# ash-shar/Long-Tail-GAN

Measured on AMD Instinct MI355X. Metric: train users/sec at BATCH_SIZE=100, higher is better.
Workload: dtype bf16

## Files before the change

long-tail-gan_amd/csrc/ltg_fast_small.h:

```cpp
#pragma once


template <bool BF>
__global__ __launch_bounds__(NT) void fk_dec1(int B, int I, int H, const float* __restrict__ h2, const float* __restrict__ Wp1t,
                                              const float* __restrict__ bp1, float* __restrict__ logits) {
    __shared__ __attribute__((aligned(16))) float lds[Rg16::LDS_FLOATS];
    const LtgTile2 tl = xcd_tile2();
    const int m0 = tl.y * 16, n0 = tl.x * 16;
    auto a_ld = [=] __device__(int, int m, int k) { return ltg_ld4(h2 + (size_t)m * H + k); };
    auto b_ld = [=] __device__(int, int k, int n) { return ltg_ld4(Wp1t + (size_t)n * H + k); };
    auto xf = [=] __device__(ltg_f32x4 v, int, int, int) { return BF ? ltg_bf16r4(v) : v; };
    const float biasv = bp1[min(n0 + (int)(threadIdx.x & 15), I - 1)];
    auto epi = [=] __device__(int, int m, int n, float v, bool ok) {
        if (ok) logits[(size_t)m * I + n] = v + biasv;
    };
    if constexpr (BF) ltg_rgemm<1, 1, 1, 1, 4, 5, true>(B, I, H, m0, n0, a_ld, xf, b_ld, xf, epi, lds);
    else ltg_rgemm<1, 1, 1, 1, 4, 10>(B, I, H, m0, n0, a_ld, xf, b_ld, xf, epi, lds);
}

__device__ __forceinline__ void block_red4(float& a, float& b, float& c, float& mx, float (*red)[NT / 64]) {
#pragma unroll
    for (int o = 32; o > 0; o >>= 1) {
        a += __shfl_xor(a, o);
        b += __shfl_xor(b, o);
        c += __shfl_xor(c, o);
        mx = fmaxf(mx, __shfl_xor(mx, o));
    }
    const int w = threadIdx.x >> 6;
    if ((threadIdx.x & 63) == 0) {
        red[0][w] = a;
        red[1][w] = b;
        red[2][w] = c;
        red[3][w] = mx;
    }
    __syncthreads();
    a = red[0][0] + red[0][1] + red[0][2] + red[0][3];
    b = red[1][0] + red[1][1] + red[1][2] + red[1][3];
    c = red[2][0] + red[2][1] + red[2][2] + red[2][3];
    mx = fmaxf(fmaxf(red[3][0], red[3][1]), fmaxf(red[3][2], red[3][3]));
    __syncthreads();
}

__global__ __launch_bounds__(NT) void fk_row_dlogits(int B, int I, const int32_t* __restrict__ indptr, const int32_t* __restrict__ indices,
                                                     const float* __restrict__ values, const float* __restrict__ logits,
                                                     const float* __restrict__ kl_rows, const float* __restrict__ y, int nf,
                                                     const int32_t* __restrict__ cnt, float lam, const int32_t* __restrict__ f_row,
                                                     const int32_t* __restrict__ f_gen, const int32_t* __restrict__ f_pop,
                                                     float* __restrict__ dlog, float* __restrict__ lse, float* __restrict__ rowout) {
    __shared__ float s_l[RD_MAXI];
    __shared__ float s_x[RD_MAXI];
    __shared__ uint8_t s_s[RD_MAXI];
    __shared__ float red[4][NT / 64];
    static_assert(NT / 64 == 4, "block_red4 adds four wave partials");
    const int b = blockIdx.x, tid = threadIdx.x;
    const float* row = logits + (size_t)b * I;
    constexpr int PER = RD_MAXI / NT;
    const int e0 = indptr[b], e1 = indptr[b + 1];
    float v[PER];
#pragma unroll
    for (int j = 0; j < PER; ++j) {
        const int i = tid + NT * j;
        v[j] = row[min(i, I - 1)];
    }
    constexpr int RD_U = 4;
    int tg0[RD_U], tr0[RD_U], tp0[RD_U];
#pragma unroll
    for (int u = 0; u < RD_U; ++u) tg0[u] = tr0[u] = tp0[u] = -1;
    if (nf > 0) {
#pragma unroll
        for (int u = 0; u < RD_U; ++u) {
            const int q = min(tid + u * NT, nf - 1);
            tg0[u] = f_gen[q];
            tr0[u] = f_row[q];
            tp0[u] = f_pop[q];
        }
    }
    const int cntv = cnt[0];
    const float klb = kl_rows[b];
    int it0 = -1;
    float x0 = 1.f;
    if (e0 + tid < e1) {
        it0 = indices[e0 + tid];
        if (values) x0 = values[e0 + tid];
    }
    float sy = 0.f;
    for (int q0 = tid; q0 < nf; q0 += RD_U * NT) {
        float ty[RD_U];
#pragma unroll
        for (int u = 0; u < RD_U; ++u) ty[u] = y[min(q0 + u * NT, nf - 1)];
#pragma unroll
        for (int u = 0; u < RD_U; ++u)
            if (q0 + u * NT < nf) sy += ty[u];
    }
    float mx = -INFINITY;
#pragma unroll
    for (int j = 0; j < PER; ++j) {
        const int i = tid + NT * j;
        if (i < I) {
            s_l[i] = v[j];
            s_x[i] = 0.f;
            s_s[i] = 0;
            mx = fmaxf(mx, v[j]);
        } else v[j] = -INFINITY;
    }
    __syncthreads();
    float xl = 0.f, nx = 0.f;
    if (it0 >= 0) {
        s_x[it0] = x0;
        xl += x0 * s_l[it0];
        nx += x0;
    }
    for (int e = e0 + tid + NT; e < e1; e += NT) {
        const int it = indices[e];
        const float x = values ? values[e] : 1.f;
        s_x[it] = x;
        xl += x * s_l[it];
        nx += x;
    }
#pragma unroll
    for (int u = 0; u < RD_U; ++u)
        if (tid + u * NT < nf && tr0[u] == b && tg0[u] >= 0 && tg0[u] < I && tp0[u] >= 0) s_s[tg0[u]] = 1;
    for (int q0 = tid + RD_U * NT; q0 < nf; q0 += RD_U * NT) {
        int tg[RD_U], tr[RD_U], tp[RD_U];
#pragma unroll
        for (int u = 0; u < RD_U; ++u) {
            const int q = min(q0 + u * NT, nf - 1);
            tg[u] = f_gen[q];
            tr[u] = f_row[q];
            tp[u] = f_pop[q];
        }
#pragma unroll
        for (int u = 0; u < RD_U; ++u)
            if (q0 + u * NT < nf && tr[u] == b && tg[u] >= 0 && tg[u] < I && tp[u] >= 0) s_s[tg[u]] = 1;
    }
    block_red4(xl, nx, sy, mx, red);
    float s = 0.f, psu = 0.f, zero = 0.f, m2 = 0.f;
#pragma unroll
    for (int j = 0; j < PER; ++j) {
        const int i = tid + NT * j;
        const float ex = expf(v[j] - mx);
        s += ex;
        psu += (i < I && s_s[i]) ? ex : 0.f;
    }
    block_red4(s, psu, zero, m2, red);
    const float l = mx + logf(s);
    const float ps = psu / s;
    const float invB = 1.f / (float)B, invs = 1.f / s;
    const float c = cntv > 0 ? lam / (float)cntv * sy : 0.f;
    const float alpha = nx * invB + c * ps;
#pragma unroll
    for (int j = 0; j < PER; ++j) {
        const int i = tid + NT * j;
        if (i < I) {
            const float p = expf(v[j] - mx) * invs;
            dlog[(size_t)b * I + i] = p * alpha - s_x[i] * invB - (s_s[i] ? c * p : 0.f);
        }
    }
    if (tid == 0) {
        lse[b] = l;
        float* o = rowout + (size_t)b * 4;
        o[0] = -xl + nx * l;
        o[1] = ps;
        o[2] = klb;
        o[3] = sy;
    }
}

constexpr int DH2_NT = 512;
template <bool BF>
__global__ __launch_bounds__(DH2_NT) void fk_dh2(int B, int I, int H, const float* __restrict__ dlog, const float* __restrict__ Wp1t,
                                             const float* __restrict__ h2, float* __restrict__ da2) {
    __shared__ __attribute__((aligned(16))) float lds[LtgRg<1, 1, 1, 1, 8>::LDS_FLOATS];
    const LtgTile2 tl = xcd_tile2();
    const int m0 = tl.y * 16, n0 = tl.x * 16;
    auto a_ld = [=] __device__(int, int m, int k) { return ltg_ld4(dlog + (size_t)m * I + k); };
    auto b_ld = [=] __device__(int, int k, int n) { return ltg_ld4s(Wp1t + (size_t)k * H + n, H); };
    auto xf = [=] __device__(ltg_f32x4 v, int, int, int) { return BF ? ltg_bf16r4(v) : v; };
    const float t = h2[(size_t)min(m0 + (int)(threadIdx.x >> 4), B - 1) * H + min(n0 + (int)(threadIdx.x & 15), H - 1)];
    auto epi = [=] __device__(int, int m, int n, float v, bool ok) {
        if (ok) da2[(size_t)m * H + n] = v * (1.f - t * t);
    };
    if constexpr (BF) ltg_rgemm<1, 1, 1, 1, 8, 4, true>(B, H, I, m0, n0, a_ld, xf, b_ld, xf, epi, lds);
    else ltg_rgemm<1, 1, 1, 1, 8, 8>(B, H, I, m0, n0, a_ld, xf, b_ld, xf, epi, lds);
}

struct WgTensors {
    float *W, *mW, *vW, *b, *mb, *vb;
};
struct WgWhere {
    float *p, *m, *v;
    bool vec;
};
struct WgRegs {
    ltg_f32x4 p, m, v;
};
#ifndef LTG_TAIL_BN
#define LTG_TAIL_BN 32
#endif
template <bool RND, bool ONES_L>
__device__ __forceinline__ void wgrad_adam_tile(int K, int Min, int Nin, const float* __restrict__ Lm, int ldl, const float* __restrict__ Rm,
                                                int ldr, WgTensors T, int ldw, AdamC ad, int m0, int n0, float* __restrict__ lds, unsigned dead = 0u) {
    const int M = ONES_L ? Min + 1 : Min, N = ONES_L ? Nin : Nin + 1;
    auto a_ld = [=] __device__(int, int m, int k) {
        ltg_f32x4 v;
#pragma unroll
        for (int j = 0; j < 4; ++j) v[j] = Lm[(size_t)min(k + j, K - 1) * ldl + min(m, Min - 1)];
        return v;
    };
    auto a_xf = [=] __device__(ltg_f32x4 x, int, int m, int k) {
        ltg_f32x4 v;
#pragma unroll
        for (int j = 0; j < 4; ++j) v[j] = k + j < K ? ((ONES_L && m == Min) ? 1.f : (RND ? ltg_bf16r(x[j]) : x[j])) : 0.f;
        return v;
    };
    auto b_ld = [=] __device__(int, int k, int n) {
        ltg_f32x4 v;
// ... 214 lines not shown
```

long-tail-gan_amd/csrc/ltg_kernels.hip:

```cpp
#include <hip/hip_runtime.h>
#include <math.h>
#include <stdint.h>

#include "../../include/ltg.h"
#include "ltg_gemm.h"
#include "ltg_rng.h"

namespace {

constexpr int NT = 256;

struct AdamC {
    float lr_t, b1, b2, eps;
};

__device__ __forceinline__ float adam_move(const float p, const float lm, const float v, const float eps) {
#ifdef LTG_ADAM_IEEE
    return p - lm / (sqrtf(v) + eps);
#else
    return __builtin_fmaf(-lm, __builtin_amdgcn_rcpf(__builtin_amdgcn_sqrtf(v) + eps), p);
#endif
}
__device__ __forceinline__ void adam1(float& p, float& m, float& v, const float g, const float lr_t, const AdamC& c) {
    m = __builtin_fmaf(c.b1, m, (1.f - c.b1) * g);
// ... 105 lines not shown
#include "ltg_diversify.h"

inline size_t align_up(size_t x, size_t a = 256) { return (x + a - 1) / a * a; }

inline bool stream_ok(const ltg_config* cfg, const ltg_gen_state* gen, int rows) {
    return gen->wp1t_bf16 && cfg->precision == LTG_PREC_BF16 && cfg->n_items >= 8192 && (cfg->n_items % 8) == 0 && rows <= 128 && cfg->h_enc <= ST_KP &&
           (cfg->h_enc % 4) == 0;
}
inline bool dw_stream_ok(int H) { return (H % 4) == 0 && H > 576 && H <= 640; }
constexpr int DH2_NH = 2;
inline int dh2_stream_chunk1(int I);
inline int dh2_stream_chunk(int I) { return DH2_NH * dh2_stream_chunk1(I); }
inline int dh2_stream_chunk1(int I) {
    int c = (I + 255) / 256;
    c = (c + ST_BN - 1) / ST_BN * ST_BN;
    return c < 4 * ST_BN ? 4 * ST_BN : c;
}

inline int dh2_kchunk(int I) {
    int chunk = (I + 63) / 64;
    chunk = (chunk + 31) / 32 * 32;
    if (chunk < 256) chunk = 256;
    return chunk;
}

inline size_t gq0_rows(const ltg_config* cfg, int ) { return (size_t)cfg->n_items; }

constexpr int RD_MAXI = 4096;
struct Workspace {
    float *rowpart, *segpart, *nb, *Pb, *scal, *dlog, *part, *dh2, *da2, *dmlv, *da1, *gq0;
    int32_t* slotmap;
    float *A1, *A3, *y, *ds, *lrow, *dpre1, *dpre3, *slab;
    float *spart, *G3, *rowout, *xd;
    uint8_t* A1_8;
    uint8_t *A1T_8, *dpre3_8, *dpre3T_8, *dpre1T_8, *ET_8;
    unsigned short* dA1T_16;
    int np8;
    float* wsp;
    size_t bytes;
};
inline int d_slab_stride(int P) { return (P + 1 + 3) & ~3; }

constexpr int FT_BM = 64, FT_NT = 512;
constexpr int FT_KP1_MAX = 4;
inline int ft_lda(int h12) { return ((h12 + 31) & ~31) + 4; }
inline size_t ft_lds_bytes(int h12) { return ((size_t)FT_BM * ft_lda(h12) + 4 * FT_BM) * sizeof(float); }
inline size_t ft_wsp_triples(int h0, int h1, int h2, int h3) {
    const size_t kp1 = (h0 + 31) / 32, kp3 = (h1 + h2 + 31) / 32;
    return (size_t)((h1 + 15) / 16) * kp1 + (size_t)((h2 + 15) / 16) * kp1 + (size_t)((h3 + 15) / 16) * kp3;
}
inline size_t ft_wsp_bytes(int h0, int h1, int h2, int h3) { return ft_wsp_triples(h0, h1, h2, h3) * 3 * 1024; }
inline bool ft_wsp_capable(const ltg_config* c) {
    return (c->tuning & 262144) == 0 && c->d_precision == LTG_PREC_FP32 && !(c->d_h0 >= 512 && c->d_h1 + c->d_h2 >= 512 && c->d_h3 >= 128) && c->d_h0 >= 4 &&
           c->d_h0 <= 32 * FT_KP1_MAX && (c->d_h0 % 4) == 0 && c->d_h1 >= 1 && c->d_h2 >= 1 && c->d_h3 >= 1 && c->d_h3 <= 320 &&
           ft_lds_bytes(c->d_h1 + c->d_h2) <= (size_t)160 * 1024;
}
Workspace carve(const ltg_config* cfg, int max_rows, int max_pairs, char* base) {
    Workspace w;
    size_t off = 0;
    auto take = [&](size_t nfloat) {
        float* p = reinterpret_cast<float*>(base + off);
        off += align_up(nfloat * sizeof(float));
        return p;
    };
    const size_t R = (size_t)max_rows, I = (size_t)cfg->n_items, H = (size_t)cfg->h_enc, Z = (size_t)cfg->z_dim;
    const size_t P = (size_t)max_pairs, h12 = (size_t)cfg->d_h1 + cfg->d_h2, h3 = (size_t)cfg->d_h3;
// ... 16 lines not shown
    w.da1 = take(R * H);
    w.gq0 = take((size_t)(gq0_rows(cfg, max_rows) + ENC0_BIAS_PARTS) * H);
    w.slotmap = reinterpret_cast<int32_t*>(take(I));
    w.A1 = take(P * h12);
    w.A3 = take(P * h3);
    w.y = take(P);
    w.ds = take(P);
    w.lrow = take(P);
    w.dpre1 = take(P * h12);
    w.dpre3 = take(P * h3);
    {
        const DLayout L = d_layout(cfg->d_h0, cfg->d_h1, cfg->d_h2, cfg->d_h3);
        const size_t ks = (P + D_KCHUNK - 1) / D_KCHUNK;
        w.slab = take(ks * (size_t)d_slab_stride(L.off[8]));
    }
    w.spart = take((((h3 + 31) / 32) + 1) * P);
    w.G3 = take(P * h3);
    w.rowout = take(R * 4);
    w.xd = take(I <= (size_t)RD_MAXI ? R * I : 1);
    w.A1_8 = reinterpret_cast<uint8_t*>(take((P * h12 + 3) / 4));
    {
        const bool f8 = cfg->d_precision == LTG_PREC_FP8;
        const size_t np = ((P + 127) / 128 * 128), h0 = (size_t)cfg->d_h0;
        auto take8 = [&](size_t nbytes) { return reinterpret_cast<uint8_t*>(take(f8 ? (nbytes + 3) / 4 : 1)); };
        w.np8 = (int)np;
        w.A1T_8 = take8((h12 + 1) * np);
        w.dA1T_16 = reinterpret_cast<unsigned short*>(take8(2 * h12 * np));
        w.dpre3_8 = take8(P * h3);
        w.dpre3T_8 = take8(h3 * np);
        w.dpre1T_8 = take8(h12 * np);
        w.ET_8 = take8(2 * (h0 + 1) * np);
    }
    w.wsp = take(ft_wsp_capable(cfg) ? ft_wsp_bytes(cfg->d_h0, cfg->d_h1, cfg->d_h2, cfg->d_h3) / sizeof(float) : 1);
    w.bytes = off;
    return w;
}

inline AdamC make_adam(const ltg_config* cfg, int t) {
    AdamC a;
    const double b1 = cfg->beta1, b2 = cfg->beta2;
    a.lr_t = (float)((double)cfg->lr * sqrt(1.0 - pow(b2, (double)t)) / (1.0 - pow(b1, (double)t)));
    a.b1 = cfg->beta1;
    a.b2 = cfg->beta2;
    a.eps = cfg->adam_eps;
    return a;
}

struct Probe {
    const ltg_probe* p;
    hipStream_t st;
    inline void before(int id) const {
        if (p && p->kernel_id == id && p->ev_start) (void)hipEventRecord((hipEvent_t)p->ev_start, st);
    }
    inline void after(int id) const {
        if (p && p->kernel_id == id && p->ev_stop) (void)hipEventRecord((hipEvent_t)p->ev_stop, st);
    }
};
#define LTG_PROBED(pr, id, stmt) \
    do {                         \
        (pr).before(id);         \
        stmt;                    \
        (pr).after(id);          \
    } while (0)

inline int check_launch() { return hipGetLastError() == hipSuccess ? LTG_OK : LTG_ELAUNCH; }
inline void clear_errors() { (void)hipGetLastError(); }
// ... 75 lines not shown
    if (fast_on(cfg)) {
        LTG_PROBED(pr, LTG_K_ENC0_FWD,
                   hipLaunchKernelGGL(fk_enc0_fwd, dim3((H / 4 + 63) / 64, R + (end_wait.word ? 1 : 0)), dim3(ENC_NT), xd ? (size_t)I * sizeof(float) : 0, st, H, I, bt->indptr,
                                      bt->indices, bt->values, o->drop_keep, o->keep_prob, cfg->seed, o->rng_step, gen->p[0], gen->p[4], acts->h1,
                                      acts->row_scale, bt->row_norm2, cfg->item_lo, Ig_of(cfg), pre_only, xd, o->rows_per_step, started, end_wait));
        return;
    }
    LTG_PROBED(pr, LTG_K_ENC0_FWD,
               hipLaunchKernelGGL(k_enc0_fwd, dim3(R), dim3(ENC_NT), (size_t)ENC_NW * H * sizeof(float), st, H, I, bt->indptr, bt->indices,
                                  bt->values, o->drop_keep, o->keep_prob, cfg->seed, o->rng_step, gen->p[0], gen->p[4], acts->h1,
                                  acts->row_scale, bt->row_norm2, cfg->item_lo, Ig_of(cfg), pre_only, o->rows_per_step));
}

int launch_dec1_fwd_stream(const ltg_config* cfg, const ltg_gen_state* gen, int R, const ltg_gen_acts* acts, float* stat, hipStream_t st) {
    const int I = cfg->n_items, H = cfg->h_enc;
    const int st2_min = (cfg->tuning & (1 << 17)) ? 8192 : ST2_MIN_ITEMS;
    if ((cfg->tuning & (1 << 26)) == 0 && I >= st2_min && (size_t)R * (size_t)I < ((size_t)1 << 30) &&
        (size_t)I * (size_t)(ST_KP * 2) < ((size_t)1 << 32)) {
        const int nt2 = (I + 31) / 32, G2 = nt2 < 256 ? nt2 : 256;
#define LTG_ST2(STATS, NTB) hipLaunchKernelGGL((k_dec1_fwd_stream2<STATS, NTB>), dim3(G2), dim3(ST_NT), (size_t)ST_KS * NTB * 64 * 16, st, R, I, H, acts->h2, gen->wp1t_bf16, gen->p[7], acts->logits, stat)
        if (stat) { if (R <= 112) LTG_ST2(true, 7); else LTG_ST2(true, 8); }
        else { if (R <= 112) LTG_ST2(false, 7); else LTG_ST2(false, 8); }
#undef LTG_ST2
        return G2;
    }
    const int ntiles = (I + ST_BN - 1) / ST_BN, G = ntiles < 256 ? ntiles : 256;
    const size_t lds = (size_t)2 * ST_BN * ST_LDW * 2;
    if (stat) hipLaunchKernelGGL(k_dec1_fwd_stream<true>, dim3(G), dim3(ST_NT), lds, st, R, I, H, acts->h2, gen->wp1t_bf16, gen->p[7], acts->logits, stat);
    else hipLaunchKernelGGL(k_dec1_fwd_stream<false>, dim3(G), dim3(ST_NT), lds, st, R, I, H, acts->h2, gen->wp1t_bf16, gen->p[7], acts->logits, (float*)nullptr);
    return G;
}

int fwd_stage_rest(const ltg_config* cfg, const ltg_gen_state* gen, const ltg_batch* bt, const ltg_fwd_opts* o,
                   const ltg_gen_acts* acts, int apply_bias_tanh, hipStream_t st, float* stat = nullptr) {
    int stat_groups = 0;
    const int R = bt->n_rows, I = cfg->n_items, H = cfg->h_enc, Z = cfg->z_dim;
    const Probe pr{o->probe, st};
    const bool vz = (Z % 4) == 0;
    if (apply_bias_tanh) {
        const int n = R * H;
        hipLaunchKernelGGL(k_bias_tanh, dim3((n + NT - 1) / NT < 1024 ? (n + NT - 1) / NT : 1024), dim3(NT), 0, st, n, H, gen->p[4], acts->h1);
    }
    if (mid_fast(cfg, R)) {
        LTG_PROBED(pr, LTG_K_ENC1, hipLaunchKernelGGL(fk_enc1<false>, grid2(Z, R, 16, 16), dim3(ENC1_NT), 0, st, R, H, Z, acts->h1, gen->p[1], gen->p[5], o->eps, o->is_training,
                                                      cfg->seed, o->rng_step, acts->mulv, acts->z));
        LTG_PROBED(pr, LTG_K_DEC0, hipLaunchKernelGGL(fk_dec0, grid2(H, R, 16, 16), dim3(NT), 0, st, R, H, Z, acts->z, acts->mulv, gen->p[2], gen->p[6],
                                                      acts->kl_rows, acts->h2));
    } else {
    pr.before(LTG_K_ENC1);
    if (vz) hipLaunchKernelGGL((k_dense_fwd<0, true>), grid2(2 * Z, R, 32, 32), dim3(NT), 0, st, R, 2 * Z, H, acts->h1, gen->p[1], gen->p[5], acts->mulv);
    else hipLaunchKernelGGL((k_dense_fwd<0, false>), grid2(2 * Z, R, 32, 32), dim3(NT), 0, st, R, 2 * Z, H, acts->h1, gen->p[1], gen->p[5], acts->mulv);
    pr.after(LTG_K_ENC1);
    hipLaunchKernelGGL(k_reparam, dim3(R), dim3(NT), 0, st, Z, acts->mulv, o->eps, o->is_training, cfg->seed, o->rng_step,
                       acts->z, acts->kl_rows);
    pr.before(LTG_K_DEC0);
    if (vz) hipLaunchKernelGGL((k_dense_fwd<1, true>), grid2(H, R, 32, 32), dim3(NT), 0, st, R, H, Z, acts->z, gen->p[2], gen->p[6], acts->h2);
    else hipLaunchKernelGGL((k_dense_fwd<1, false>), grid2(H, R, 32, 32), dim3(NT), 0, st, R, H, Z, acts->z, gen->p[2], gen->p[6], acts->h2);
    pr.after(LTG_K_DEC0);
    }
    {
        const bool bf = cfg->precision == LTG_PREC_BF16, big = I >= 8192;
        pr.before(LTG_K_DEC1_FWD);
        if (fast_on(cfg) && I <= RD_MAXI && R <= 256) {
            if (bf) hipLaunchKernelGGL(fk_dec1<true>, grid2(I, R, 16, 16), dim3(NT), 0, st, R, I, H, acts->h2, gen->p[3], gen->p[7], acts->logits);
            else hipLaunchKernelGGL(fk_dec1<false>, grid2(I, R, 16, 16), dim3(NT), 0, st, R, I, H, acts->h2, gen->p[3], gen->p[7], acts->logits);
        } else if (stream_ok(cfg, gen, R)) {
            if (stat && (cfg->tuning & (1 << 21)) == 0)
                stat_groups = launch_dec1_fwd_stream(cfg, gen, R, acts, stat, st);
            else
                launch_dec1_fwd_stream(cfg, gen, R, acts, nullptr, st);
        } else if (bf && big) hipLaunchKernelGGL((k_dec1_fwd<true, true>), grid2(I, R, 64, 128), dim3(NT), 0, st, R, I, H, acts->h2, gen->p[3], gen->p[7], acts->logits);
        else if (bf) hipLaunchKernelGGL((k_dec1_fwd<true, false, true>), grid2(I, R, 32, 32), dim3(NT), 0, st, R, I, H, acts->h2, gen->p[3], gen->p[7], acts->logits);
        else if (big) hipLaunchKernelGGL((k_dec1_fwd<false, true>), grid2(I, R, 64, 128), dim3(NT), 0, st, R, I, H, acts->h2, gen->p[3], gen->p[7], acts->logits);
        else hipLaunchKernelGGL((k_dec1_fwd<false, false>), grid2(I, R, 32, 32), dim3(NT), 0, st, R, I, H, acts->h2, gen->p[3], gen->p[7], acts->logits);
        pr.after(LTG_K_DEC1_FWD);
    }
    return stat_groups;
}

inline size_t segpart_bytes(const ltg_config* cfg, int rows) {
    return align_up((size_t)rows * RP * sizeof(float)) + align_up(segpart_floats(cfg->n_items, rows) * sizeof(float));
}

int vae_forward_impl(const ltg_config* cfg, const ltg_gen_state* gen, const ltg_batch* bt, const ltg_fwd_opts* o,
                     const ltg_gen_acts* acts, float* probs_out, hipStream_t st, void* ws = nullptr, size_t ws_bytes = 0) {
    const int R = bt->n_rows, I = cfg->n_items;
    if (R <= 0) return LTG_OK;
    fwd_stage_enc(cfg, gen, bt, o, acts, 0, st);
    const bool have_scratch = ws && I > 2 * RS_SEG && ws_bytes >= segpart_bytes(cfg, R);
    float* segpart = have_scratch ? reinterpret_cast<float*>((char*)ws + align_up((size_t)R * RP * sizeof(float))) : nullptr;
    const int sg = fwd_stage_rest(cfg, gen, bt, o, acts, 0, st, segpart);
    if (sg > 0) {
        hipLaunchKernelGGL(k_row_stats_merge, dim3(R), dim3(NT), 0, st, R, sg, I, cfg->item_lo, segpart, bt->indptr, bt->indices, bt->values, acts->logits, 0,
                           (const int32_t*)nullptr, (const int32_t*)nullptr, (const int32_t*)nullptr, (float*)nullptr, acts->lse);
    } else if (have_scratch) {
        const int nseg = (I + RS_SEG - 1) / RS_SEG;
        hipLaunchKernelGGL(k_row_partial_seg, dim3(nseg, R), dim3(NT), 0, st, I, cfg->item_lo, bt->indptr, bt->indices, bt->values, acts->logits,
                           0, (const int32_t*)nullptr, (const int32_t*)nullptr, (const int32_t*)nullptr, segpart);
// ... 624 lines not shown

int ltg_g_step(const ltg_config* cfg, const ltg_gen_state* gen, const ltg_disc_state* disc, const ltg_batch* bt,
               const ltg_pairs* fake, const ltg_g_opts* o, const ltg_gen_acts* acts, float* loss_out, void* ws,
               size_t ws_bytes, ltg_stream stream) {
    clear_errors();
    if (!cfg_ok(cfg) || !gen || !disc || !bt || !fake || !o || !acts || !loss_out || !ws || o->adam_t < 1) return LTG_EINVAL;
    if (!bt->uptr || !bt->rowidx || !bt->csr_pos || !o->cnt || !fake->row || bt->n_rows <= 0 || fake->n < 0) return LTG_EINVAL;
    if (bt->n_unique < 0 || (size_t)bt->n_unique > gq0_rows(cfg, bt->n_rows)) return LTG_EINVAL;
    const int B = bt->n_rows, nf = fake->n;
    if (ltg_workspace_bytes(cfg, B, nf) > ws_bytes) return LTG_EWORKSPACE;
    hipStream_t st = (hipStream_t)stream;
    Workspace w = carve(cfg, B, nf, (char*)ws);
    const bool have_y = o->y_pre != nullptr;
    if (have_y) w.y = const_cast<float*>(o->y_pre);
    q0_touch(cfg, gen, bt, st);
    const bool aux_sweep = q0_lazy(cfg, gen) && o->aux_stream && o->ev_fork && o->ev_sweep;
    const bool fork = o->aux_stream && o->ev_fork && o->ev_join && nf > 0 && !have_y;
    if (fork || aux_sweep) {
        hipStream_t aux = (hipStream_t)o->aux_stream;
        if (hipEventRecord((hipEvent_t)o->ev_fork, st) != hipSuccess || hipStreamWaitEvent(aux, (hipEvent_t)o->ev_fork, 0) != hipSuccess)
            return LTG_ELAUNCH;
        if (fork) {
            PairView pv{0, nf, nullptr, nullptr, fake->pop, fake->niche};
            DropView dA{nullptr, o->drop_fake[0], 0, 0}, dB{nullptr, o->drop_fake[1], 0, 0}, dC{nullptr, o->drop_fake[2], 0, 0};
            disc_forward(cfg, disc, pv, dA, dB, dC, o->d_keep_prob, o->d_rng_step, w, false, nullptr, aux);
            if (hipEventRecord((hipEvent_t)o->ev_join, aux) != hipSuccess) return LTG_ELAUNCH;
        }
    }
    ltg_g_opts o_local = *o;
    o_local.fake_done = (o->fake_done & 1) | (aux_sweep ? G_AUX_SWEEP : 0);
    o = &o_local;
    const bool small = small_fast(cfg, B);
    fwd_stage_enc(cfg, gen, bt, &o->fwd, acts, 0, st, small ? w.xd : nullptr, true);
    const int sgroups = fwd_stage_rest(cfg, gen, bt, &o->fwd, acts, 0, st, small ? nullptr : w.segpart);
    if (small) {
        const int I = cfg->n_items, H = cfg->h_enc;
        const Probe pr{o->probe, st};
        if (nf > 0 && !fork && !have_y) {
            PairView pv{0, nf, nullptr, nullptr, fake->pop, fake->niche};
            DropView dA{nullptr, o->drop_fake[0], 0, 0}, dB{nullptr, o->drop_fake[1], 0, 0}, dC{nullptr, o->drop_fake[2], 0, 0};
            disc_forward(cfg, disc, pv, dA, dB, dC, o->d_keep_prob, o->d_rng_step, w, false, o->probe, st);
        }
        if (fork && hipStreamWaitEvent(st, (hipEvent_t)o->ev_join, 0) != hipSuccess) return LTG_ELAUNCH;
        LTG_PROBED(pr, LTG_K_ROW_DLOGITS, hipLaunchKernelGGL(fk_row_dlogits, dim3(B), dim3(NT), 0, st, B, I, bt->indptr, bt->indices, bt->values, acts->logits,
                                                             acts->kl_rows, w.y, nf, o->cnt, o->gan_lambda, fake->row, fake->niche, fake->pop, w.dlog,
                                                             acts->lse, w.rowout));
        pr.before(LTG_K_DH2);
        if (cfg->precision == LTG_PREC_BF16) hipLaunchKernelGGL(fk_dh2<true>, grid2(H, B, 16, 16), dim3(DH2_NT), 0, st, B, I, H, w.dlog, gen->p[3], acts->h2, w.da2);
        else hipLaunchKernelGGL(fk_dh2<false>, grid2(H, B, 16, 16), dim3(DH2_NT), 0, st, B, I, H, w.dlog, gen->p[3], acts->h2, w.da2);
        pr.after(LTG_K_DH2);
        g_chain(cfg, gen, bt, o, acts, w, make_adam(cfg, o->adam_t), nullptr, true, loss_out, st);
        return check_launch();
    }
    g_row_partial(cfg, bt, fake, acts, w.rowpart, st, w.segpart, nullptr, sgroups);
    if (fork && hipStreamWaitEvent(st, (hipEvent_t)o->ev_join, 0) != hipSuccess) return LTG_ELAUNCH;
    int rc = g_stage_bwd_dec(cfg, gen, disc, bt, fake, o, acts, w.rowpart, 1, loss_out, w, w.da2, st, fork || have_y, acts->h2);
    if (rc != LTG_OK) return rc;
    rc = g_stage_bwd_rest(cfg, gen, bt, o, acts, w.da2, w, st, true);
    if (aux_sweep && hipStreamWaitEvent(st, (hipEvent_t)o->ev_sweep, 0) != hipSuccess) return LTG_ELAUNCH;
    return rc;
}

int ltg_g_fwd_enc(const ltg_config* cfg, const ltg_gen_state* gen, const ltg_batch* bt, const ltg_fwd_opts* opts,
                  const ltg_gen_acts* acts, ltg_stream stream) {
    clear_errors();
    if (!g_args_ok(cfg, gen, bt, acts) || !opts) return LTG_EINVAL;
    fwd_stage_enc(cfg, gen, bt, opts, acts, 1, (hipStream_t)stream);
    return check_launch();
}

int ltg_g_fwd_rest(const ltg_config* cfg, const ltg_gen_state* gen, const ltg_batch* bt, const ltg_pairs* fake,
                   const ltg_fwd_opts* opts, const ltg_gen_acts* acts, float* rowpart_out, void* ws, size_t ws_bytes,
                   ltg_stream stream) {
    clear_errors();
    if (!g_args_ok(cfg, gen, bt, acts) || !opts || !rowpart_out) return LTG_EINVAL;
    hipStream_t st = (hipStream_t)stream;
    float* segpart = (ws && ws_bytes >= segpart_bytes(cfg, bt->n_rows))
                         ? reinterpret_cast<float*>((char*)ws + align_up((size_t)bt->n_rows * RP * sizeof(float))) : nullptr;
    const int sgroups = fwd_stage_rest(cfg, gen, bt, opts, acts, 1, st, segpart);
    g_row_partial(cfg, bt, (fake && fake->n > 0) ? fake : nullptr, acts, rowpart_out, st, segpart, nullptr, sgroups);
    return check_launch();
}
// ... 579 lines not shown
```

Measured before the change: 86540.

## Fuse row softmax/dlogits into dh2 GEMM using per-tile stats from decoder forward

The decoder forward kernel now also writes per-16-column tile max and exp-sum statistics. The separate fk_row_dlogits kernel is removed, and fk_dh2 computes the row softmax statistics, the positive and fake-item maps (in an LDS bitmap) and the dlogits values on the fly inside its A-operand transform. Column-0 tiles write dlog, lse and rowout. This saves one kernel launch and a round trip of dlog through global memory. In exchange, every dh2 block redundantly rebuilds the row statistics and maps, and the shared-memory footprint is larger.

```diff
diff --git a/long-tail-gan_amd/csrc/ltg_fast_small.h b/long-tail-gan_amd/csrc/ltg_fast_small.h
--- a/long-tail-gan_amd/csrc/ltg_fast_small.h
+++ b/long-tail-gan_amd/csrc/ltg_fast_small.h
@@ -1,9 +1,9 @@
 #pragma once
 
 
-template <bool BF>
+template <bool BF, bool ST = false>
 __global__ __launch_bounds__(NT) void fk_dec1(int B, int I, int H, const float* __restrict__ h2, const float* __restrict__ Wp1t,
-                                              const float* __restrict__ bp1, float* __restrict__ logits) {
+                                              const float* __restrict__ bp1, float* __restrict__ logits, float* __restrict__ tstat = nullptr) {
     __shared__ __attribute__((aligned(16))) float lds[Rg16::LDS_FLOATS];
     const LtgTile2 tl = xcd_tile2();
     const int m0 = tl.y * 16, n0 = tl.x * 16;
@@ -12,176 +12,257 @@
     auto xf = [=] __device__(ltg_f32x4 v, int, int, int) { return BF ? ltg_bf16r4(v) : v; };
     const float biasv = bp1[min(n0 + (int)(threadIdx.x & 15), I - 1)];
     auto epi = [=] __device__(int, int m, int n, float v, bool ok) {
-        if (ok) logits[(size_t)m * I + n] = v + biasv;
+        const float x = v + biasv;
+        if (ok) logits[(size_t)m * I + n] = x;
+        if constexpr (ST) {
+            float tm = n < I ? x : -INFINITY;
+#pragma unroll
+            for (int o = 8; o > 0; o >>= 1) tm = fmaxf(tm, __shfl_xor(tm, o));
+            float te = n < I ? expf(x - tm) : 0.f;
+#pragma unroll
+            for (int o = 8; o > 0; o >>= 1) te += __shfl_xor(te, o);
+            if ((threadIdx.x & 15) == 0 && m < B) *reinterpret_cast<float2*>(tstat + ((size_t)m * gridDim.x + tl.x) * 2) = make_float2(tm, te);
+        }
     };
     if constexpr (BF) ltg_rgemm<1, 1, 1, 1, 4, 5, true>(B, I, H, m0, n0, a_ld, xf, b_ld, xf, epi, lds);
     else ltg_rgemm<1, 1, 1, 1, 4, 10>(B, I, H, m0, n0, a_ld, xf, b_ld, xf, epi, lds);
 }
 
-__device__ __forceinline__ void block_red4(float& a, float& b, float& c, float& mx, float (*red)[NT / 64]) {
-#pragma unroll
-    for (int o = 32; o > 0; o >>= 1) {
-        a += __shfl_xor(a, o);
-        b += __shfl_xor(b, o);
-        c += __shfl_xor(c, o);
-        mx = fmaxf(mx, __shfl_xor(mx, o));
-    }
-    const int w = threadIdx.x >> 6;
-    if ((threadIdx.x & 63) == 0) {
-        red[0][w] = a;
-        red[1][w] = b;
-        red[2][w] = c;
-        red[3][w] = mx;
-    }
-    __syncthreads();
-    a = red[0][0] + red[0][1] + red[0][2] + red[0][3];
-    b = red[1][0] + red[1][1] + red[1][2] + red[1][3];
-    c = red[2][0] + red[2][1] + red[2][2] + red[2][3];
-    mx = fmaxf(fmaxf(red[3][0], red[3][1]), fmaxf(red[3][2], red[3][3]));
-    __syncthreads();
-}
-
-__global__ __launch_bounds__(NT) void fk_row_dlogits(int B, int I, const int32_t* __restrict__ indptr, const int32_t* __restrict__ indices,
-                                                     const float* __restrict__ values, const float* __restrict__ logits,
-                                                     const float* __restrict__ kl_rows, const float* __restrict__ y, int nf,
-                                                     const int32_t* __restrict__ cnt, float lam, const int32_t* __restrict__ f_row,
-                                                     const int32_t* __restrict__ f_gen, const int32_t* __restrict__ f_pop,
-                                                     float* __restrict__ dlog, float* __restrict__ lse, float* __restrict__ rowout) {
-    __shared__ float s_l[RD_MAXI];
-    __shared__ float s_x[RD_MAXI];
-    __shared__ uint8_t s_s[RD_MAXI];
-    __shared__ float red[4][NT / 64];
-    static_assert(NT / 64 == 4, "block_red4 adds four wave partials");
-    const int b = blockIdx.x, tid = threadIdx.x;
-    const float* row = logits + (size_t)b * I;
-    constexpr int PER = RD_MAXI / NT;
-    const int e0 = indptr[b], e1 = indptr[b + 1];
-    float v[PER];
-#pragma unroll
-    for (int j = 0; j < PER; ++j) {
-        const int i = tid + NT * j;
-        v[j] = row[min(i, I - 1)];
-    }
-    constexpr int RD_U = 4;
-    int tg0[RD_U], tr0[RD_U], tp0[RD_U];
-#pragma unroll
-    for (int u = 0; u < RD_U; ++u) tg0[u] = tr0[u] = tp0[u] = -1;
-    if (nf > 0) {
-#pragma unroll
-        for (int u = 0; u < RD_U; ++u) {
-            const int q = min(tid + u * NT, nf - 1);
-            tg0[u] = f_gen[q];
-            tr0[u] = f_row[q];
-            tp0[u] = f_pop[q];
-        }
-    }
-    const int cntv = cnt[0];
-    const float klb = kl_rows[b];
-    int it0 = -1;
-    float x0 = 1.f;
-    if (e0 + tid < e1) {
-        it0 = indices[e0 + tid];
-        if (values) x0 = values[e0 + tid];
-    }
-    float sy = 0.f;
-    for (int q0 = tid; q0 < nf; q0 += RD_U * NT) {
-        float ty[RD_U];
-#pragma unroll
-        for (int u = 0; u < RD_U; ++u) ty[u] = y[min(q0 + u * NT, nf - 1)];
-#pragma unroll
-        for (int u = 0; u < RD_U; ++u)
-            if (q0 + u * NT < nf) sy += ty[u];
-    }
-    float mx = -INFINITY;
-#pragma unroll
-    for (int j = 0; j < PER; ++j) {
-        const int i = tid + NT * j;
-        if (i < I) {
-            s_l[i] = v[j];
-            s_x[i] = 0.f;
-            s_s[i] = 0;
-            mx = fmaxf(mx, v[j]);
-        } else v[j] = -INFINITY;
-    }
-    __syncthreads();
-    float xl = 0.f, nx = 0.f;
-    if (it0 >= 0) {
-        s_x[it0] = x0;
-        xl += x0 * s_l[it0];
-        nx += x0;
-    }
-    for (int e = e0 + tid + NT; e < e1; e += NT) {
-        const int it = indices[e];
-        const float x = values ? values[e] : 1.f;
-        s_x[it] = x;
-        xl += x * s_l[it];
-        nx += x;
-    }
-#pragma unroll
-    for (int u = 0; u < RD_U; ++u)
-        if (tid + u * NT < nf && tr0[u] == b && tg0[u] >= 0 && tg0[u] < I && tp0[u] >= 0) s_s[tg0[u]] = 1;
-    for (int q0 = tid + RD_U * NT; q0 < nf; q0 += RD_U * NT) {
-        int tg[RD_U], tr[RD_U], tp[RD_U];
-#pragma unroll
-        for (int u = 0; u < RD_U; ++u) {
-            const int q = min(q0 + u * NT, nf - 1);
-            tg[u] = f_gen[q];
-            tr[u] = f_row[q];
-            tp[u] = f_pop[q];
-        }
-#pragma unroll
-        for (int u = 0; u < RD_U; ++u)
-            if (q0 + u * NT < nf && tr[u] == b && tg[u] >= 0 && tg[u] < I && tp[u] >= 0) s_s[tg[u]] = 1;
-    }
-    block_red4(xl, nx, sy, mx, red);
-    float s = 0.f, psu = 0.f, zero = 0.f, m2 = 0.f;
-#pragma unroll
-    for (int j = 0; j < PER; ++j) {
-        const int i = tid + NT * j;
-        const float ex = expf(v[j] - mx);
-        s += ex;
-        psu += (i < I && s_s[i]) ? ex : 0.f;
-    }
-    block_red4(s, psu, zero, m2, red);
-    const float l = mx + logf(s);
-    const float ps = psu / s;
-    const float invB = 1.f / (float)B, invs = 1.f / s;
-    const float c = cntv > 0 ? lam / (float)cntv * sy : 0.f;
-    const float alpha = nx * invB + c * ps;
-#pragma unroll
-    for (int j = 0; j < PER; ++j) {
-        const int i = tid + NT * j;
-        if (i < I) {
-            const float p = expf(v[j] - mx) * invs;
-            dlog[(size_t)b * I + i] = p * alpha - s_x[i] * invB - (s_s[i] ? c * p : 0.f);
-        }
-    }
-    if (tid == 0) {
-        lse[b] = l;
-        float* o = rowout + (size_t)b * 4;
-        o[0] = -xl + nx * l;
-        o[1] = ps;
-        o[2] = klb;
-        o[3] = sy;
-    }
-}
-
 constexpr int DH2_NT = 512;
-template <bool BF>
-__global__ __launch_bounds__(DH2_NT) void fk_dh2(int B, int I, int H, const float* __restrict__ dlog, const float* __restrict__ Wp1t,
-                                             const float* __restrict__ h2, float* __restrict__ da2) {
-    __shared__ __attribute__((aligned(16))) float lds[LtgRg<1, 1, 1, 1, 8>::LDS_FLOATS];
+constexpr int RD_U = 4;
+constexpr int DH2_TS_U = 2;
+constexpr int DH2_CS_U = 4;
+constexpr int DH2_XOFF = 0x1FFF;
+constexpr unsigned DH2_SBIT = 0x8000u;
+constexpr int DH2_ROW_FLOATS = 96;
+inline size_t dh2_lds_bytes(int I) { return (size_t)(LtgRg<1, 1, 1, 1, 8>::LDS_FLOATS + DH2_ROW_FLOATS) * sizeof(float) + (size_t)16 * I * 2; }
+constexpr int DH2_ONE_I = 1024;
+template <bool BF, bool ONE>
+__global__ __launch_bounds__(DH2_NT, ONE ? 4 : 2) void fk_dh2(int B, int I, int H, const float* __restrict__ logits, const float* __restrict__ tstat,
+                                                 const int32_t* __restrict__ indptr, const int32_t* __restrict__ indices, const float* __restrict__ values,
+                                                 const float* __restrict__ kl_rows, const float* __restrict__ y, int nf, const int32_t* __restrict__ cnt,
+                                                 float lam, const int32_t* __restrict__ f_row, const int32_t* __restrict__ f_gen,
+                                                 const int32_t* __restrict__ f_pop, const float* __restrict__ Wp1t, const float* __restrict__ h2,
+                                                 float* __restrict__ da2, float* __restrict__ dlog, float* __restrict__ lse, float* __restrict__ rowout) {
+    extern __shared__ __attribute__((aligned(16))) float dh2_lds[];
+    if constexpr (ONE) __builtin_assume(I <= DH2_ONE_I);
+    constexpr int PROD = LtgRg<1, 1, 1, 1, 8>::LDS_FLOATS;
+    static_assert((PROD + DH2_ROW_FLOATS) % 4 == 0, "the map starts on 16 bytes");
+    float* lds = dh2_lds;
+    float* s_mx = dh2_lds + PROD;
+    float* s_invs = s_mx + 16;
+    float* s_alpha = s_invs + 16;
+    float* s_red = s_alpha + 16;
+    int* s_e0 = reinterpret_cast<int*>(s_red + 8);
+    int* s_e1 = s_e0 + 16;
+    unsigned* map32 = reinterpret_cast<unsigned*>(dh2_lds + PROD + DH2_ROW_FLOATS);
+    const unsigned short* map16 = reinterpret_cast<const unsigned short*>(map32);
     const LtgTile2 tl = xcd_tile2();
     const int m0 = tl.y * 16, n0 = tl.x * 16;
-    auto a_ld = [=] __device__(int, int m, int k) { return ltg_ld4(dlog + (size_t)m * I + k); };
+    const int tid = threadIdx.x;
+    const bool writer = tl.x == 0;
+    const int nct = (I + 15) >> 4;
+    const float invB = 1.f / (float)B;
+    const int rr = tid >> 5, j = tid & 31;
+    const bool rowok = m0 + rr < B;
+    const int rowc = min(m0 + rr, B - 1);
+    float2 ts[DH2_TS_U];
+#pragma unroll
+    for (int u = 0; u < DH2_TS_U; ++u) ts[u] = *reinterpret_cast<const float2*>(tstat + (rowc * nct + min(j + 32 * u, nct - 1)) * 2);
+    const int32_t* fg = nf > 0 ? f_gen : cnt;
+    const int32_t* fr = nf > 0 ? f_row : cnt;
+    const int32_t* fp = nf > 0 ? f_pop : cnt;
+    const float* fy = nf > 0 ? y : kl_rows;
+    int tg0[RD_U], tr0[RD_U], tp0[RD_U];
+    float ty0[RD_U];
+#pragma unroll
+    for (int u = 0; u < RD_U; ++u) {
+        const int q = max(min(tid + u * DH2_NT, nf - 1), 0);
+        tg0[u] = fg[q];
+        tr0[u] = fr[q];
+        tp0[u] = fp[q];
+        ty0[u] = fy[q];
+    }
+    const int cntv = cnt[0];
+    const int e0 = indptr[rowc];
+    const int e1r = indptr[rowc + 1];
+    const bool lane_rowok = m0 + (tid & 15) < B;
+    float t = 0.f, klb = 0.f;
+    float a_mx = 0.f, a_invs = 0.f, a_alpha = 0.f, c = 0.f;
+    constexpr int DH2_NREQ = 8;
+    static_assert(DH2_NREQ == (BF ? 2 * 4 : 8), "NBLK of the ltg_rgemm call below");
+    const int Kc = (I - 1) & ~3;
+    const int lrow = min(m0 + (tid & 15), B - 1);
+    ltg_f32x4 av[DH2_NREQ];
+    bool a_have = false;
+    auto req_a = [&] __device__(int k0) {
+#pragma unroll
+        for (int ii = 0; ii < DH2_NREQ; ++ii) av[ii] = ltg_ld4(logits + lrow * I + min(k0 + (BF ? 32 * (ii >> 1) + 4 * (ii & 1) : 16 * ii), Kc));
+    };
+    auto mid = [&] __device__() {
+        t = h2[(size_t)min(m0 + (int)(threadIdx.x >> 4), B - 1) * H + min(n0 + (int)(threadIdx.x & 15), H - 1)];
+        klb = kl_rows[rowc];
+        {
+            const uint4 z = make_uint4(0u, 0u, 0u, 0u);
+            uint4* m4 = reinterpret_cast<uint4*>(map32);
+            for (int i = tid; i < 2 * I; i += DH2_NT) m4[i] = z;
+        }
+        float mx = -INFINITY, s = 0.f;
+        auto merge = [&] __device__(float2 p) {
+            const float nm = fmaxf(mx, p.x);
+            s = s * expf(mx - nm) + p.y * expf(p.x - nm);
+            mx = nm;
+        };
+#pragma unroll
+        for (int u = 0; u < DH2_TS_U; ++u)
+            if (j + 32 * u < nct) merge(ts[u]);
+#pragma unroll 1
+        for (int tt = j + 32 * DH2_TS_U; tt < nct; tt += 32) merge(*reinterpret_cast<const float2*>(tstat + (rowc * nct + tt) * 2));
+        __syncthreads();
+        float sy = 0.f;
+        auto mark = [&] __device__(int q, int tg, int tr, int tp, float yv) {
+            if (q < nf) {
+                sy += yv;
+                const int d = tr - m0;
+                if (d >= 0 && d < 16 && tr < B && tg >= 0 && tg < I && tp >= 0) atomicOr(&map32[(d * I + tg) >> 1], DH2_SBIT << (16 * (tg & 1)));
+            }
+        };
+#pragma unroll
+        for (int u = 0; u < RD_U; ++u) mark(tid + u * DH2_NT, tg0[u], tr0[u], tp0[u], ty0[u]);
+#pragma unroll 1
+        for (int q0 = tid + RD_U * DH2_NT; q0 < nf; q0 += RD_U * DH2_NT) {
+            int tg[RD_U], tr[RD_U], tp[RD_U];
+            float ty[RD_U];
+#pragma unroll
+            for (int u = 0; u < RD_U; ++u) {
+                const int q = min(q0 + u * DH2_NT, nf - 1);
+                tg[u] = f_gen[q];
+                tr[u] = f_row[q];
+                tp[u] = f_pop[q];
+                ty[u] = y[q];
+            }
+#pragma unroll
+            for (int u = 0; u < RD_U; ++u) mark(q0 + u * DH2_NT, tg[u], tr[u], tp[u], ty[u]);
+        }
+        float nx = 0.f, xl = 0.f;
+        const int e1 = rowok ? e1r : e0;
+#pragma unroll 1
+        for (int eb = e0 + j; eb < e1; eb += 32 * DH2_CS_U) {
+            int it[DH2_CS_U];
+            float xv[DH2_CS_U], lg[DH2_CS_U];
+#pragma unroll
+            for (int u = 0; u < DH2_CS_U; ++u) {
+                const int e = min(eb + 32 * u, e1 - 1);
+                it[u] = indices[e];
+                xv[u] = values ? values[e] : 1.f;
+            }
+#pragma unroll
+            for (int u = 0; u < DH2_CS_U; ++u) {
+                it[u] = (eb + 32 * u < e1 && it[u] >= 0 && it[u] < I) ? it[u] : -1;
+                lg[u] = 0.f;
+            }
+            if (writer) {
+#pragma unroll
+                for (int u = 0; u < DH2_CS_U; ++u) lg[u] = logits[rowc * I + max(it[u], 0)];
+            }
+#pragma unroll
+            for (int u = 0; u < DH2_CS_U; ++u)
+                if (it[u] >= 0) {
+                    const unsigned off = (unsigned)min(eb + 32 * u - e0 + 1, DH2_XOFF);
+                    atomicOr(&map32[(rr * I + it[u]) >> 1], off << (16 * (it[u] & 1)));
+                    nx += xv[u];
+                    xl += xv[u] * lg[u];
+                }
+        }
+#pragma unroll
+        for (int o = 32; o > 0; o >>= 1) sy += __shfl_xor(sy, o);
+        if ((tid & 63) == 0) s_red[tid >> 6] = sy;
+        float M = mx;
+#pragma unroll
+        for (int o = 16; o > 0; o >>= 1) M = fmaxf(M, __shfl_xor(M, o));
+        s *= expf(mx - M);
+#pragma unroll
+        for (int o = 16; o > 0; o >>= 1) {
+            s += __shfl_xor(s, o);
+            nx += __shfl_xor(nx, o);
+            xl += __shfl_xor(xl, o);
+        }
+        __syncthreads();
+        float syt = s_red[0];
+#pragma unroll
+        for (int w = 1; w < DH2_NT / 64; ++w) syt += s_red[w];
+        c = cntv > 0 ? lam / (float)cntv * syt : 0.f;
+        float psu = 0.f;
+        if (nf > 0) {
+#pragma unroll 1
+            for (int i4 = 4 * j; i4 < I; i4 += 128) {
+                const uint2 hw = *reinterpret_cast<const uint2*>(map16 + rr * I + i4);
+                if ((hw.x | hw.y) & (DH2_SBIT | (DH2_SBIT << 16))) {
+                    const ltg_f32x4 l4 = ltg_ld4(logits + rowc * I + i4);
+                    psu += (hw.x & DH2_SBIT) ? expf(l4[0] - M) : 0.f;
+                    psu += (hw.x & (DH2_SBIT << 16)) ? expf(l4[1] - M) : 0.f;
+                    psu += (hw.y & DH2_SBIT) ? expf(l4[2] - M) : 0.f;
+                    psu += (hw.y & (DH2_SBIT << 16)) ? expf(l4[3] - M) : 0.f;
+                }
+            }
+#pragma unroll
+            for (int o = 16; o > 0; o >>= 1) psu += __shfl_xor(psu, o);
+        }
+        const float ps = psu / s;
+        {
+            constexpr int BLK = BF ? 32 : 16;
+            const int per = (((I + BLK - 1) / BLK) + DH2_NT / 64 - 1) / (DH2_NT / 64);
+            req_a(min(BLK * ((tid >> 6) * per) + (BLK / 4) * ((tid & 63) >> 4), Kc));
+            a_have = true;
+        }
+        if (j == 0) {
+            s_e0[rr] = e0;
+            s_e1[rr] = e1r;
+            s_mx[rr] = M;
+            s_invs[rr] = 1.f / s;
+            s_alpha[rr] = nx * invB + c * ps;
+            if (writer && rowok) {
+                const float l = M + logf(s);
+                lse[m0 + rr] = l;
+                float* o = rowout + (m0 + rr) * 4;
+                o[0] = -xl + nx * l;
+                o[1] = ps;
+                o[2] = klb;
+                o[3] = syt;
+            }
+        }
+        __syncthreads();
+        a_mx = s_mx[tid & 15];
+        a_invs = s_invs[tid & 15];
+        a_alpha = s_alpha[tid & 15];
+    };
+    auto a_ld = [=] __device__(int, int, int) { return 0; };
+    auto a_xf = [&] __device__(int, int i, int m, int k) {
+        if (i == 0) {
+            if (!a_have) req_a(k);
+            a_have = false;
+        }
+        const uint2 hw = *reinterpret_cast<const uint2*>(map16 + (tid & 15) * I + k);
+        const ltg_f32x4 v = av[i];
+        ltg_f32x4 d;
+#pragma unroll
+        for (int jj = 0; jj < 4; ++jj) {
+            const unsigned h = ((jj < 2 ? hw.x : hw.y) >> (16 * (jj & 1))) & 0xFFFFu;
+            const float p = expf(v[jj] - a_mx) * a_invs;
+            float x = 0.f;
+            if (h & DH2_XOFF) x = values ? values[min(s_e0[tid & 15] + (int)(h & DH2_XOFF) - 1, s_e1[tid & 15] - 1)] : 1.f;
+            d[jj] = p * a_alpha - x * invB - ((h & DH2_SBIT) ? c * p : 0.f);
+        }
+        if (writer && lane_rowok) *reinterpret_cast<ltg_f32x4*>(dlog + m * I + k) = d;
+        return BF ? ltg_bf16r4(d) : d;
+    };
     auto b_ld = [=] __device__(int, int k, int n) { return ltg_ld4s(Wp1t + (size_t)k * H + n, H); };
-    auto xf = [=] __device__(ltg_f32x4 v, int, int, int) { return BF ? ltg_bf16r4(v) : v; };
-    const float t = h2[(size_t)min(m0 + (int)(threadIdx.x >> 4), B - 1) * H + min(n0 + (int)(threadIdx.x & 15), H - 1)];
-    auto epi = [=] __device__(int, int m, int n, float v, bool ok) {
+    auto b_xf = [=] __device__(ltg_f32x4 v, int, int, int) { return BF ? ltg_bf16r4(v) : v; };
+    auto epi = [&] __device__(int, int m, int n, float v, bool ok) {
         if (ok) da2[(size_t)m * H + n] = v * (1.f - t * t);
     };
-    if constexpr (BF) ltg_rgemm<1, 1, 1, 1, 8, 4, true>(B, H, I, m0, n0, a_ld, xf, b_ld, xf, epi, lds);
-    else ltg_rgemm<1, 1, 1, 1, 8, 8>(B, H, I, m0, n0, a_ld, xf, b_ld, xf, epi, lds);
+    if constexpr (BF) ltg_rgemm<1, 1, 1, 1, 8, 4, true, true>(B, H, I, m0, n0, a_ld, a_xf, b_ld, b_xf, epi, lds, mid);
+    else ltg_rgemm<1, 1, 1, 1, 8, 8, false, true>(B, H, I, m0, n0, a_ld, a_xf, b_ld, b_xf, epi, lds, mid);
 }
 
 struct WgTensors {
diff --git a/long-tail-gan_amd/csrc/ltg_kernels.hip b/long-tail-gan_amd/csrc/ltg_kernels.hip
--- a/long-tail-gan_amd/csrc/ltg_kernels.hip
+++ b/long-tail-gan_amd/csrc/ltg_kernels.hip
@@ -161,6 +161,7 @@
     int32_t* slotmap;
     float *A1, *A3, *y, *ds, *lrow, *dpre1, *dpre3, *slab;
     float *spart, *G3, *rowout, *xd;
+    float* tstat;
     uint8_t* A1_8;
     uint8_t *A1T_8, *dpre3_8, *dpre3T_8, *dpre1T_8, *ET_8;
     unsigned short* dA1T_16;
@@ -243,6 +244,7 @@
         w.ET_8 = take8(2 * (h0 + 1) * np);
     }
     w.wsp = take(ft_wsp_capable(cfg) ? ft_wsp_bytes(cfg->d_h0, cfg->d_h1, cfg->d_h2, cfg->d_h3) / sizeof(float) : 1);
+    w.tstat = take(I <= (size_t)RD_MAXI ? R * ((I + 15) / 16) * 2 : 1);
     w.bytes = off;
     return w;
 }
@@ -384,7 +386,7 @@
 }
 
 int fwd_stage_rest(const ltg_config* cfg, const ltg_gen_state* gen, const ltg_batch* bt, const ltg_fwd_opts* o,
-                   const ltg_gen_acts* acts, int apply_bias_tanh, hipStream_t st, float* stat = nullptr) {
+                   const ltg_gen_acts* acts, int apply_bias_tanh, hipStream_t st, float* stat = nullptr, float* tile_stat = nullptr) {
     int stat_groups = 0;
     const int R = bt->n_rows, I = cfg->n_items, H = cfg->h_enc, Z = cfg->z_dim;
     const Probe pr{o->probe, st};
@@ -414,8 +416,10 @@
         const bool bf = cfg->precision == LTG_PREC_BF16, big = I >= 8192;
         pr.before(LTG_K_DEC1_FWD);
         if (fast_on(cfg) && I <= RD_MAXI && R <= 256) {
-            if (bf) hipLaunchKernelGGL(fk_dec1<true>, grid2(I, R, 16, 16), dim3(NT), 0, st, R, I, H, acts->h2, gen->p[3], gen->p[7], acts->logits);
-            else hipLaunchKernelGGL(fk_dec1<false>, grid2(I, R, 16, 16), dim3(NT), 0, st, R, I, H, acts->h2, gen->p[3], gen->p[7], acts->logits);
+            if (tile_stat && bf) hipLaunchKernelGGL((fk_dec1<true, true>), grid2(I, R, 16, 16), dim3(NT), 0, st, R, I, H, acts->h2, gen->p[3], gen->p[7], acts->logits, tile_stat);
+            else if (tile_stat) hipLaunchKernelGGL((fk_dec1<false, true>), grid2(I, R, 16, 16), dim3(NT), 0, st, R, I, H, acts->h2, gen->p[3], gen->p[7], acts->logits, tile_stat);
+            else if (bf) hipLaunchKernelGGL((fk_dec1<true, false>), grid2(I, R, 16, 16), dim3(NT), 0, st, R, I, H, acts->h2, gen->p[3], gen->p[7], acts->logits, (float*)nullptr);
+            else hipLaunchKernelGGL((fk_dec1<false, false>), grid2(I, R, 16, 16), dim3(NT), 0, st, R, I, H, acts->h2, gen->p[3], gen->p[7], acts->logits, (float*)nullptr);
         } else if (stream_ok(cfg, gen, R)) {
             if (stat && (cfg->tuning & (1 << 21)) == 0)
                 stat_groups = launch_dec1_fwd_stream(cfg, gen, R, acts, stat, st);
@@ -1106,7 +1110,7 @@
     o = &o_local;
     const bool small = small_fast(cfg, B);
     fwd_stage_enc(cfg, gen, bt, &o->fwd, acts, 0, st, small ? w.xd : nullptr, true);
-    const int sgroups = fwd_stage_rest(cfg, gen, bt, &o->fwd, acts, 0, st, small ? nullptr : w.segpart);
+    const int sgroups = fwd_stage_rest(cfg, gen, bt, &o->fwd, acts, 0, st, small ? nullptr : w.segpart, small ? w.tstat : nullptr);
     if (small) {
         const int I = cfg->n_items, H = cfg->h_enc;
         const Probe pr{o->probe, st};
@@ -1116,12 +1120,13 @@
             disc_forward(cfg, disc, pv, dA, dB, dC, o->d_keep_prob, o->d_rng_step, w, false, o->probe, st);
         }
         if (fork && hipStreamWaitEvent(st, (hipEvent_t)o->ev_join, 0) != hipSuccess) return LTG_ELAUNCH;
-        LTG_PROBED(pr, LTG_K_ROW_DLOGITS, hipLaunchKernelGGL(fk_row_dlogits, dim3(B), dim3(NT), 0, st, B, I, bt->indptr, bt->indices, bt->values, acts->logits,
-                                                             acts->kl_rows, w.y, nf, o->cnt, o->gan_lambda, fake->row, fake->niche, fake->pop, w.dlog,
-                                                             acts->lse, w.rowout));
         pr.before(LTG_K_DH2);
-        if (cfg->precision == LTG_PREC_BF16) hipLaunchKernelGGL(fk_dh2<true>, grid2(H, B, 16, 16), dim3(DH2_NT), 0, st, B, I, H, w.dlog, gen->p[3], acts->h2, w.da2);
-        else hipLaunchKernelGGL(fk_dh2<false>, grid2(H, B, 16, 16), dim3(DH2_NT), 0, st, B, I, H, w.dlog, gen->p[3], acts->h2, w.da2);
+#define LTG_DH2(BFV, ONEV)                                                                                                                                   \
+    hipLaunchKernelGGL((fk_dh2<BFV, ONEV>), grid2(H, B, 16, 16), dim3(DH2_NT), dh2_lds_bytes(I), st, B, I, H, acts->logits, w.tstat, bt->indptr, bt->indices, bt->values, \
+                       acts->kl_rows, w.y, nf, o->cnt, o->gan_lambda, fake->row, fake->niche, fake->pop, gen->p[3], acts->h2, w.da2, w.dlog, acts->lse, w.rowout)
+        if (cfg->precision == LTG_PREC_BF16) { if (I <= DH2_ONE_I) LTG_DH2(true, true); else LTG_DH2(true, false); }
+        else { if (I <= DH2_ONE_I) LTG_DH2(false, true); else LTG_DH2(false, false); }
+#undef LTG_DH2
         pr.after(LTG_K_DH2);
         g_chain(cfg, gen, bt, o, acts, w, make_adam(cfg, o->adam_t), nullptr, true, loss_out, st);
         return check_launch();
```

After: 81810. -5.5%, worse.
